# jgaeddert/liquid-usrp

Hardware: AMD Instinct MI355X
Metric: complex Msamples/s through multichannelrx (higher is better)
Workload: dtype f32

## Files before the change

### liquid-usrp_amd/csrc/lean_prims.hpp

```cpp
#pragma once
namespace lean {

typedef float v2f __attribute__((ext_vector_type(2)));
__device__ __forceinline__ v2f cmul_pk(v2f a, v2f tw)
{
    v2f t, r;
    asm("v_pk_mul_f32 %0, %1, %2 op_sel_hi:[1,0]" : "=v"(t) : "v"(a), "v"(tw));
    asm("v_pk_fma_f32 %0, %1, %2, %3 op_sel:[1,1,0] op_sel_hi:[0,1,1] neg_lo:[1,0,0]" : "=v"(r) : "v"(a), "v"(tw), "v"(t));
    return r;
}
__device__ __forceinline__ v2f cmulc_pk(v2f a, v2f tw)
{
    v2f t, r;
    asm("v_pk_mul_f32 %0, %1, %2 op_sel_hi:[1,0]" : "=v"(t) : "v"(a), "v"(tw));
    asm("v_pk_fma_f32 %0, %1, %2, %3 op_sel:[1,1,0] op_sel_hi:[0,1,1] neg_hi:[1,0,0]" : "=v"(r) : "v"(a), "v"(tw), "v"(t));
    return r;
}
__device__ __forceinline__ v2f rot_down_pk(v2f a, float rev)
{
    v2f cs; cs.x = __builtin_amdgcn_cosf(rev); cs.y = __builtin_amdgcn_sinf(rev);
    return cmulc_pk(a, cs);
}
template <int HI>
__device__ __forceinline__ v2f bfly_pk(v2f x, v2f sgp, v2f p)
{
    v2f r;
    if constexpr (HI == 0) asm("v_pk_fma_f32 %0, %1, %2, %3 op_sel_hi:[1,0,1]" : "=v"(r) : "v"(x), "v"(sgp), "v"(p));
    else                   asm("v_pk_fma_f32 %0, %1, %2, %3 op_sel:[0,1,0] op_sel_hi:[1,1,1]" : "=v"(r) : "v"(x), "v"(sgp), "v"(p));
    return r;
}

template <int H>
__device__ __forceinline__ float xch(float v, int bp32)
{
    if constexpr (H == 32) return __builtin_bit_cast(float, __builtin_amdgcn_ds_bpermute(bp32, __builtin_bit_cast(int, v)));
    else return __builtin_bit_cast(float, __builtin_amdgcn_ds_swizzle(__builtin_bit_cast(int, v), (H << 10) | 0x1F));
}
template <int H, int XB, int HI>
__device__ __forceinline__ v2f stage(v2f x, v2f sgp, v2f tw, int bp32)
{
    v2f u;
    if constexpr ((XB & H) != 0) { v2f p; p.x = xch<H>(x.x, bp32); p.y = xch<H>(x.y, bp32); u = bfly_pk<HI>(x, sgp, p); }
    else { const float sg = HI ? sgp.y : sgp.x; u.x = bfly_leg<H>(x.x, sg); u.y = bfly_leg<H>(x.y, sg); }
    if constexpr (H == 1) return u;
    else return cmul_pk(u, tw);
}


template <int MM> __device__ __forceinline__ int lane_k(int l)
{
    if constexpr (MM == 64) return (int)(__brev((unsigned)l) >> 26);
    else return l < 48 ? (l >> 4) + 3 * (int)(__brev((unsigned)(l & 15)) >> 28) : -1;
}
template <int MM> __device__ __forceinline__ int k_lane(int k)
{
    if constexpr (MM == 64) return (int)(__brev((unsigned)k) >> 26);
    else return 16 * (k % 3) + (int)(__brev((unsigned)(k / 3)) >> 28);
}
struct Radix3 { v2f w1, w2, t; int a0, a1, a2; };
__device__ __forceinline__ Radix3 radix3_consts(int l)
{
    Radix3 r;
    const int a = l >> 4, b = l & 15;
    const float r1 = (float)(a % 3) * (1.0f / 3.0f), r2 = (float)((2 * a) % 3) * (1.0f / 3.0f), rt = (float)(b * (a % 3)) * (1.0f / 48.0f);
    r.w1.x = __builtin_amdgcn_cosf(r1); r.w1.y = -__builtin_amdgcn_sinf(r1);
    r.w2.x = __builtin_amdgcn_cosf(r2); r.w2.y = -__builtin_amdgcn_sinf(r2);
    r.t.x = __builtin_amdgcn_cosf(rt);  r.t.y = -__builtin_amdgcn_sinf(rt);
    r.a0 = b << 2; r.a1 = (16 + b) << 2; r.a2 = (32 + b) << 2;
    return r;
}
template <int XB>
__device__ __forceinline__ v2f fft48(v2f x, const v2f (&tw)[6], const v2f (&sgp)[3], const Radix3 &r3, int bp32, int l)
{
    const float xr = x.x, xi = x.y;
    v2f x0, x1, x2;
    x0.x = __builtin_bit_cast(float, __builtin_amdgcn_ds_bpermute(r3.a0, __builtin_bit_cast(int, xr)));
    x0.y = __builtin_bit_cast(float, __builtin_amdgcn_ds_bpermute(r3.a0, __builtin_bit_cast(int, xi)));
    x1.x = __builtin_bit_cast(float, __builtin_amdgcn_ds_bpermute(r3.a1, __builtin_bit_cast(int, xr)));
    x1.y = __builtin_bit_cast(float, __builtin_amdgcn_ds_bpermute(r3.a1, __builtin_bit_cast(int, xi)));
    x2.x = __builtin_bit_cast(float, __builtin_amdgcn_ds_bpermute(r3.a2, __builtin_bit_cast(int, xr)));
    x2.y = __builtin_bit_cast(float, __builtin_amdgcn_ds_bpermute(r3.a2, __builtin_bit_cast(int, xi)));
    const v2f p1 = cmul_pk(x1, r3.w1), p2 = cmul_pk(x2, r3.w2);
    v2f y; y.x = (x0.x + p1.x) + p2.x; y.y = (x0.y + p1.y) + p2.y;
    y = cmul_pk(y, r3.t);
    if (l >= 48) { y.x = 0.f; y.y = 0.f; }
    y = stage<8, XB, 0>(y, sgp[1], tw[2], bp32);
    y = stage<4, XB, 1>(y, sgp[1], tw[3], bp32);
    y = stage<2, XB, 0>(y, sgp[2], tw[4], bp32);
    y = stage<1, XB, 1>(y, sgp[2], tw[5], bp32);
    return y;
}
template <int XB>
__device__ __forceinline__ v2f fft64(v2f x, const v2f (&tw)[6], const v2f (&sgp)[3], int bp32)
{
    x = stage<32, XB, 0>(x, sgp[0], tw[0], bp32);
    x = stage<16, XB, 1>(x, sgp[0], tw[1], bp32);
    x = stage<8, XB, 0>(x, sgp[1], tw[2], bp32);
    x = stage<4, XB, 1>(x, sgp[1], tw[3], bp32);
    x = stage<2, XB, 0>(x, sgp[2], tw[4], bp32);
    x = stage<1, XB, 1>(x, sgp[2], tw[5], bp32);
    return x;
}

}
```

### liquid-usrp_amd/csrc/payload_lean.hpp

```cpp

#ifndef PL_NT_STORE
#define PL_NT_STORE 0
#endif
#include "lean_prims.hpp"
#include "demod_pk.hpp"
namespace lean {

template <int MOD, int XB, int MM = 64>
__device__ __forceinline__ uint32_t symbols(const SyncArgs &a, const PayloadJob *job, const uint32_t ch, const uint32_t j,
                                            const uint32_t *qsg, const uint32_t *qnb, const int *qsrc)
{
    constexpr unsigned bps = bits_per_symbol<MOD>::v;
    const SyncConsts &c = a.c;
    const int l = lane_id();
    const int bp32 = (l ^ 32) << 2;
    const int kq = lane_k<MM>(l);
    const bool lane_on = kq >= 0;
    const int kk = lane_on ? kq : 0;
    const int dr = lane_on ? c.data_rank[kk] : -1;
    const bool isdata = dr >= 0;
    Radix3 r3; if constexpr (MM == 48) r3 = radix3_consts(l);
    const float fxr = ((kk > c.M2) ? (float)kk - (float)c.M : (float)kk) * 0.15915494309189535f;
    v2f R = {0.f, 0.f};
    if (lane_on && c.sctype[kk]) { const float2 g = (a.jR + (size_t)j * c.M)[kk]; R.x = g.x; R.y = g.y; }
    v2f tw[6], sgp[3];
#pragma unroll
    for (int st = 0; st < 6; st++) {
        const int h = 32 >> st;
        const bool up = (l & h) != 0;
        const float rev = (float)(l & (h - 1)) * (0.5f / (float)h);
        tw[st].x = up ? __builtin_amdgcn_cosf(rev) : 1.f; tw[st].y = up ? -__builtin_amdgcn_sinf(rev) : 0.f;
        if (st & 1) sgp[st >> 1].y = up ? -1.f : 1.f; else sgp[st >> 1].x = up ? -1.f : 1.f;
    }
    const int Mp = c.M_pilot;
    const bool p8 = Mp <= 8;
    const float pf0 = (l < Mp) ? c.Pfit[l] : 0.f, pf1 = (l < Mp) ? c.Pfit[Mp + l] : 0.f;
    const float pfc = p8 ? ((l < 8) ? pf0 : ((l < 16 && l - 8 < Mp) ? c.Pfit[Mp + l - 8] : 0.f)) : pf0;
    const int psrc = qsrc[l < Mp ? l : 0] << 2;
    const uint32_t so_sym = (uint32_t)(isdata ? dr : 0) * 8u, so_soft = (uint32_t)(isdata ? dr : 0) * bps;

    const int L = c.L, cb = c.cp - c.backoff, Md = c.M_data;
    const uint32_t mod_len = rfl(job->s.mod_len), nbits = rfl(8u * job->s.enc_len);
    const uint32_t nsym = (mod_len + (uint32_t)Md - 1u) / (uint32_t)Md;
    const int64_t t_ev0 = job->s.cur + (int64_t)job->s.timer - 1;
    const int64_t ws0 = t_ev0 - L + 1 + cb;
    uint32_t dth = rfl(job->s.nco_dtheta);
    uint32_t th_ws = rfl(job->s.nco_theta_ref + (uint32_t)(ws0 - job->s.nco_t_ref) * job->s.nco_dtheta);
    uint32_t pc4 = rfl(job->s.pilot_count) * 4u;
    float phi_prime = job->s.phi_prime, p1_prime = job->s.p1_prime;
    int32_t r_ws = (int32_t)rfl((uint32_t)(ws0 - a.buf_first));
    const float2 *chb = a.chan + ((size_t)a.chan_off + ch) * MCRX_TILE_S;
    const uint32_t tstride = a.chan_stride * (uint32_t)MCRX_TILE_S;
    const int32_t r_max = (int32_t)(a.end - a.buf_first) - 1;
    const bool soft_mode = c.payload_soft != 0;
    const bool keep_syms = a.no_syms == 0;
    uint8_t *soft = a.jsoft + (size_t)j * 8 * c.max_enc_len;
    const uint64_t syms_off = job->syms_off;
    uint8_t *syms = a.sarena + (((uint64_t)rfl((uint32_t)(syms_off >> 32)) << 32) | rfl((uint32_t)syms_off));
    const uint32_t l4 = (uint32_t)l * 4u;

    int q0 = -1, q1 = -1; uint32_t offl = 0, offl1 = 0;
    auto load_win = [&](int32_t rw) -> v2f {
        if (rw >= 0 && rw + (WV - 1) <= r_max) {
            const int ph = rw & (MCRX_TILE_S - 1);
            if (ph != q0) {
                const int tq = q0; const uint32_t to = offl; q0 = q1; offl = offl1; q1 = tq; offl1 = to;
                if (ph != q0) { q0 = ph; const uint32_t q = (uint32_t)ph + (uint32_t)l; offl = ((q >> MCRX_TILE_SH) * tstride + (q & (uint32_t)(MCRX_TILE_S - 1))) * 8u; }
            }
            const char *base = reinterpret_cast<const char *>(chb + (size_t)(uint32_t)(rw >> MCRX_TILE_SH) * tstride);
            v2f v = *reinterpret_cast<const v2f *>(base + offl);
            if constexpr (MM < WV) { if (l >= MM) { v.x = 0.f; v.y = 0.f; } }
            return v;
        }
        int32_t r = rw + l;
        r = r < 0 ? 0 : (r > r_max ? r_max : r);
        v2f v = *reinterpret_cast<const v2f *>(chb + ((size_t)(r >> MCRX_TILE_SH) * tstride + (size_t)(r & (MCRX_TILE_S - 1))));
        if constexpr (MM < WV) { if (l >= MM) { v.x = 0.f; v.y = 0.f; } }
        return v;
    };

    auto store_symbol = [&](uint32_t ps, v2f Z, uint64_t sw, bool inner) {
        uint8_t *ssym = syms + (size_t)ps * 8, *ssoft = soft + (size_t)ps * bps;
        if (inner || (ps + (uint32_t)Md <= mod_len && (ps + (uint32_t)Md) * bps <= nbits)) {
            if (isdata) {
#if PL_NT_STORE
                if (keep_syms) __builtin_nontemporal_store(Z, reinterpret_cast<v2f *>(ssym + so_sym));
#else
                if (keep_syms) *reinterpret_cast<v2f *>(ssym + so_sym) = Z;
#endif
                uint8_t *dst = ssoft + so_soft;
                if constexpr (bps == 1) dst[0] = (uint8_t)sw;
                else if constexpr (bps == 2) *reinterpret_cast<uint16_t *>(dst) = (uint16_t)sw;
                else {
                    *reinterpret_cast<uint16_t *>(dst) = (uint16_t)sw;
                    *reinterpret_cast<uint16_t *>(dst + 2) = (uint16_t)(sw >> 16);
                    if constexpr (bps == 6) *reinterpret_cast<uint16_t *>(dst + 4) = (uint16_t)(sw >> 32);
                }
            }
        } else if (isdata && ps + (uint32_t)dr < mod_len) {
            if (keep_syms) *reinterpret_cast<v2f *>(ssym + so_sym) = Z;
            const uint32_t b0 = (ps + (uint32_t)dr) * bps;
#pragma unroll
            for (unsigned kb = 0; kb < bps; kb++) if (b0 + kb < nbits) ssoft[so_soft + kb] = (uint8_t)(sw >> (8 * kb));
        }
    };
    v2f cur = load_win(r_ws);
    v2f Zp = {0.f, 0.f}; uint64_t swp = 0;
    uint32_t psi = 0;
    for (uint32_t n = 0; n < nsym; n++) {
        const uint32_t sgn = *reinterpret_cast<const uint32_t *>(reinterpret_cast<const char *>(qsg) + (pc4 + (l < 16 ? l4 : 0u)));
        v2f x = rot_down_pk(cur, u32rev(th_ws + (uint32_t)l * dth));
        if (n + 1 < nsym) cur = load_win(r_ws + L);
        if (n > 0) store_symbol(psi - (uint32_t)Md, Zp, swp, true);
        if constexpr (MM == 64) x = fft64<XB>(x, tw, sgp, bp32);
        else x = fft48<XB>(x, tw, sgp, r3, bp32, l);
        x = cmul_pk(x, R);
        const float xr = x.x, xi = x.y;
        float2 P;
        P.x = __builtin_bit_cast(float, __builtin_amdgcn_ds_bpermute(psrc, __builtin_bit_cast(int, xr)) ^ (int)sgn);
        P.y = __builtin_bit_cast(float, __builtin_amdgcn_ds_bpermute(psrc, __builtin_bit_cast(int, xi)) ^ (int)sgn);
        const float v = atan2_fast(P.y, P.x);
        const float prev = dpp_mov<0x111, false>(v, v);
        const float turns = rintf((v - prev) * 0.15915494309189535f);
        float p0, p1;
        if (p8) {
            float t = turns;
            t += dpp_mov<0x111>(t); t += dpp_mov<0x112>(t); t += dpp_mov<0x114>(t);
            const float y = fmaf(-TWO_PI_F, t, v);
            const int yi = __builtin_bit_cast(int, y);
            float z = pfc * __builtin_bit_cast(float, __builtin_amdgcn_update_dpp(yi, yi, 0x118, 0xf, 0xc, false));
            z += dpp_mov<0x111>(z); z += dpp_mov<0x112>(z); z += dpp_mov<0x114>(z);
            p0 = __builtin_bit_cast(float, __builtin_amdgcn_readlane(__builtin_bit_cast(int, z), 7));
            p1 = __builtin_bit_cast(float, __builtin_amdgcn_readlane(__builtin_bit_cast(int, z), 15));
        } else {
            const float y = fmaf(-TWO_PI_F, row_scan_fast(turns), v);
            p0 = row_total_dpp(pf0 * y);
            p1 = row_total_dpp(pf1 * y);
        }
        pc4 += (uint32_t)Mp * 4u; pc4 = pc4 >= 255u * 4u ? pc4 - 255u * 4u : pc4;
        p1 = 0.3f * p1 + (1.0f - 0.3f) * p1_prime;
        p1_prime = p1;
        Zp = rot_down_pk(x, fmaf(p1, fxr, p0 * 0.15915494309189535f));
        swp = demod_pk<MOD>(reinterpret_cast<const uint8_t *>(qnb), Zp, soft_mode);
        psi += (uint32_t)Md;
        float dphi = p0 - phi_prime;
        dphi -= TWO_PI_F * rintf(dphi * 0.15915494309189535f);
        phi_prime = p0;
        const uint32_t dnew = dth + rfl((uint32_t)__float2int_rn(dphi * (1e-3f * 683565275.5764316f)));
        th_ws += (uint32_t)(L - cb) * dth + (uint32_t)cb * dnew;
        dth = dnew;
        r_ws += L;
    }
    if (nsym > 0) store_symbol(psi - (uint32_t)Md, Zp, swp, false);
    return dth;
}

}

template <int XB, int CLS, bool REST = false, int MM = 64>
__device__ __forceinline__ void payload_lean_body(SyncArgs &a)
{
    launder(a);
    __shared__ uint32_t qsg[256 + 16];
    __shared__ uint32_t qnb[64];
    __shared__ int qsrc[16];
    const SyncConsts &c = a.c;
    const int l = lane_id();
    const uint32_t nj = a.max_jobs;
    uint32_t nlist = (CLS == 1 && a.qam_list) ? a.qam_list[0] : a.live[0];
    if (nlist > nj) nlist = nj;
    const uint32_t kfirst = REST ? a.live_off + blockIdx.x : blockIdx.x;
    if (kfirst >= nlist) return;
    for (int k = l; k < 256 + 16; k += WV) qsg[k] = c.pilot_seq[k >= 255 ? k - 255 : k] == 0 ? 0x80000000u : 0u;
    if (l < 16) qsrc[l] = 0;
    wave_sync_lds();
    { const int kq = lean::lane_k<MM>(l); const int pr = kq >= 0 ? c.pilot_rank[kq] : -1; if (pr >= 0 && pr < 16) qsrc[pr] = l; }
    wave_sync_lds();
    for (uint32_t k = kfirst; k < nlist; k += gridDim.x) {
        const uint32_t j = (CLS == 1 && a.qam_list) ? rfl(a.qam_list[1 + k]) : rfl(a.live[1 + k]);
        if (j >= nj) continue;
        const PayloadJob *job = a.jobs + j;
        const uint32_t ch = rfl(job->ch);
        if (ch >= a.nch || job->arena_off == ~0ull) continue;
        const uint32_t mod = rfl(job->s.mod_scheme);
        if (((mod == 39 || mod == 40) ? 0 : 1) != CLS) continue;
        uint32_t dth;
        if constexpr (CLS == 0) {
            if (mod == 39) dth = lean::symbols<39, XB, MM>(a, job, ch, j, qsg, qnb, qsrc);
            else           dth = lean::symbols<40, XB, MM>(a, job, ch, j, qsg, qnb, qsrc);
        } else {
            wave_sync_lds();
            if (mod == 27) { if (l < 16) qnb[l] = reinterpret_cast<const uint32_t *>(c.cod.qam16_nb)[l]; }
            else qnb[l] = reinterpret_cast<const uint32_t *>(c.cod.qam64_nb)[l];
            wave_sync_lds();
            if (mod == 27) dth = lean::symbols<27, XB, MM>(a, job, ch, j, qsg, qnb, qsrc);
            else           dth = lean::symbols<29, XB, MM>(a, job, ch, j, qsg, qnb, qsrc);
        }
        if (l == 0) a.jobs[j].s.nco_dtheta = dth;
        if (CLS == 0 && !REST) break;
    }
}
template <int XB, int MM = 64> __global__ __launch_bounds__(WV) __attribute__((amdgpu_num_sgpr(72))) void payload_lean_kernel(SyncArgs a) { payload_lean_body<XB, 0, false, MM>(a); }
template <int XB, int MM = 64> __global__ __launch_bounds__(WV) void payload_lean_rest_kernel(SyncArgs a) { payload_lean_body<XB, 0, true, MM>(a); payload_lean_body<XB, 1, false, MM>(a); }
```

### liquid-usrp_amd/csrc/payload_wide.hpp

```cpp
#include "lean_prims.hpp"
#include "demod_pk.hpp"
namespace lean {

template <int MOD, int XB, int E>
__device__ __forceinline__ uint32_t symbols_wide(const SyncArgs &a, const PayloadJob *job, const uint32_t ch, const uint32_t j,
                                                 const uint32_t *qsg, const uint32_t *qnb, const int *qsrc)
{
    constexpr unsigned bps = MOD == 39 ? 1u : MOD == 40 ? 2u : MOD == 27 ? 4u : 6u;
    constexpr int LOG2E = E == 2 ? 1 : (E == 4 ? 2 : 3);
    static_assert(E == 2 || E == 4 || E == 8, "symbol widths 128, 256, 512");
    const SyncConsts &c = a.c;
    const int l = lane_id();
    const int bp32 = (l ^ 32) << 2;
    int dr[E]; float fxr[E]; v2f R[E]; uint32_t so_sym[E], so_soft[E];
#pragma unroll
    for (int e = 0; e < E; e++) {
        const int kk = (int)(__brev((unsigned)(l + WV * e)) >> (32 - 6 - LOG2E));
        dr[e] = c.data_rank[kk];
        fxr[e] = ((kk > c.M2) ? (float)kk - (float)c.M : (float)kk) * 0.15915494309189535f;
        R[e].x = 0.f; R[e].y = 0.f;
        if (c.sctype[kk]) { const float2 g = (a.jR + (size_t)j * c.M)[kk]; R[e].x = g.x; R[e].y = g.y; }
        so_sym[e] = (uint32_t)(dr[e] >= 0 ? dr[e] : 0) * 8u; so_soft[e] = (uint32_t)(dr[e] >= 0 ? dr[e] : 0) * bps;
    }
    v2f tw[6], sgp[3];
#pragma unroll
    for (int st = 0; st < 6; st++) {
        const int h = 32 >> st;
        const bool up = (l & h) != 0;
        const float rev = (float)(l & (h - 1)) * (0.5f / (float)h);
        tw[st].x = up ? __builtin_amdgcn_cosf(rev) : 1.f; tw[st].y = up ? -__builtin_amdgcn_sinf(rev) : 0.f;
        if (st & 1) sgp[st >> 1].y = up ? -1.f : 1.f; else sgp[st >> 1].x = up ? -1.f : 1.f;
    }
    v2f itw[E - 1];
#pragma unroll
    for (int J = E / 2; J >= 1; J >>= 1)
#pragma unroll
        for (int r = 0; r < J; r++) {
            const float rev = (float)(l + WV * r) * (0.5f / (float)(WV * J));
            itw[J - 1 + r].x = __builtin_amdgcn_cosf(rev); itw[J - 1 + r].y = __builtin_amdgcn_sinf(rev);
        }
    const int Mp = c.M_pilot;
    const float pf0 = (l < Mp) ? c.Pfit[l] : 0.f, pf1 = (l < Mp) ? c.Pfit[Mp + l] : 0.f;
    const int psrc = qsrc[l < Mp ? l : 0];
    const int paddr = (psrc & 63) << 2, pel = psrc >> 8;

    const int L = c.L, cb = c.cp - c.backoff, Md = c.M_data;
    const uint32_t mod_len = rfl(job->s.mod_len), nbits = rfl(8u * job->s.enc_len);
    const uint32_t nsym = (mod_len + (uint32_t)Md - 1u) / (uint32_t)Md;
    const int64_t t_ev0 = job->s.cur + (int64_t)job->s.timer - 1;
    const int64_t ws0 = t_ev0 - L + 1 + cb;
    uint32_t dth = rfl(job->s.nco_dtheta);
    uint32_t th_ws = rfl(job->s.nco_theta_ref + (uint32_t)(ws0 - job->s.nco_t_ref) * job->s.nco_dtheta);
    uint32_t pc4 = rfl(job->s.pilot_count) * 4u;
    float phi_prime = job->s.phi_prime, p1_prime = job->s.p1_prime;
    int32_t r_ws = (int32_t)rfl((uint32_t)(ws0 - a.buf_first));
    const float2 *chb = a.chan + ((size_t)a.chan_off + ch) * MCRX_TILE_S;
    const uint32_t tstride = a.chan_stride * (uint32_t)MCRX_TILE_S;
    const int32_t r_max = (int32_t)(a.end - a.buf_first) - 1;
    const bool soft_mode = c.payload_soft != 0;
    const bool keep_syms = a.no_syms == 0;
    uint8_t *soft = a.jsoft + (size_t)j * 8 * c.max_enc_len;
    const uint64_t syms_off = job->syms_off;
    uint8_t *syms = a.sarena + (((uint64_t)rfl((uint32_t)(syms_off >> 32)) << 32) | rfl((uint32_t)syms_off));
    const uint32_t l4 = (uint32_t)l * 4u;

    int q0 = -1; uint32_t offl = 0;
    const uint32_t estep = (uint32_t)(WV >> MCRX_TILE_SH) * tstride * 8u;
    auto load_win = [&](int32_t rw, v2f (&w)[E]) {
        if (rw >= 0 && rw + (WV * E - 1) <= r_max) {
            const int ph = rw & (MCRX_TILE_S - 1);
            if (ph != q0) { q0 = ph; const uint32_t q = (uint32_t)ph + (uint32_t)l; offl = ((q >> MCRX_TILE_SH) * tstride + (q & (uint32_t)(MCRX_TILE_S - 1))) * 8u; }
            const char *base = reinterpret_cast<const char *>(chb + (size_t)(uint32_t)(rw >> MCRX_TILE_SH) * tstride) + offl;
#pragma unroll
            for (int e = 0; e < E; e++) w[e] = *reinterpret_cast<const v2f *>(base + (size_t)e * estep);
            return;
        }
#pragma unroll
        for (int e = 0; e < E; e++) {
            int32_t r = rw + l + WV * e;
            r = r < 0 ? 0 : (r > r_max ? r_max : r);
            w[e] = *reinterpret_cast<const v2f *>(chb + ((size_t)(r >> MCRX_TILE_SH) * tstride + (size_t)(r & (MCRX_TILE_S - 1))));
        }
    };
    auto store_symbol = [&](uint32_t ps, const v2f (&Z)[E], const uint64_t (&sw)[E], bool inner) {
        uint8_t *ssym = syms + (size_t)ps * 8, *ssoft = soft + (size_t)ps * bps;
        const bool whole = inner || (ps + (uint32_t)Md <= mod_len && (ps + (uint32_t)Md) * bps <= nbits);
#pragma unroll
        for (int e = 0; e < E; e++) {
            if (dr[e] < 0) continue;
            if (whole) {
                if (keep_syms) *reinterpret_cast<v2f *>(ssym + so_sym[e]) = Z[e];
                uint8_t *dst = ssoft + so_soft[e];
                if constexpr (bps == 1) dst[0] = (uint8_t)sw[e];
                else if constexpr (bps == 2) *reinterpret_cast<uint16_t *>(dst) = (uint16_t)sw[e];
                else if constexpr (bps == 4) *reinterpret_cast<uint32_t *>(dst) = (uint32_t)sw[e];
                else {
                    *reinterpret_cast<uint16_t *>(dst) = (uint16_t)sw[e];
                    *reinterpret_cast<uint16_t *>(dst + 2) = (uint16_t)(sw[e] >> 16);
                    *reinterpret_cast<uint16_t *>(dst + 4) = (uint16_t)(sw[e] >> 32);
                }
            } else if (ps + (uint32_t)dr[e] < mod_len) {
                if (keep_syms) *reinterpret_cast<v2f *>(ssym + so_sym[e]) = Z[e];
                const uint32_t b0 = (ps + (uint32_t)dr[e]) * bps;
#pragma unroll
                for (unsigned kb = 0; kb < bps; kb++) if (b0 + kb < nbits) ssoft[so_soft[e] + kb] = (uint8_t)(sw[e] >> (8 * kb));
            }
        }
    };
    v2f cur[E];
    load_win(r_ws, cur);
    v2f Zp[E]; uint64_t swp[E];
#pragma unroll
    for (int e = 0; e < E; e++) { Zp[e].x = 0.f; Zp[e].y = 0.f; swp[e] = 0; }
    uint32_t psi = 0;
    for (uint32_t n = 0; n < nsym; n++) {
        const uint32_t sgn = *reinterpret_cast<const uint32_t *>(reinterpret_cast<const char *>(qsg) + (pc4 + (l < Mp ? l4 : 0u)));
        v2f x[E];
#pragma unroll
        for (int e = 0; e < E; e++) x[e] = rot_down_pk(cur[e], u32rev(th_ws + (uint32_t)(l + WV * e) * dth));
        if (n + 1 < nsym) load_win(r_ws + L, cur);
        if (n > 0) store_symbol(psi - (uint32_t)Md, Zp, swp, true);
#pragma unroll
        for (int J = E / 2; J >= 1; J >>= 1)
#pragma unroll
            for (int e = 0; e < E; e++)
                if ((e & J) == 0) {
                    const v2f u = x[e], v = x[e + J];
                    x[e] = u + v;
                    x[e + J] = cmulc_pk(u - v, itw[J - 1 + (e & (J - 1))]);
                }
#pragma unroll
        for (int e = 0; e < E; e++) { x[e] = fft64<XB>(x[e], tw, sgp, bp32); x[e] = cmul_pk(x[e], R[e]); }
        float px = 0.f, py = 0.f;
#pragma unroll
        for (int e = 0; e < E; e++) {
            const float xr = x[e].x, xi = x[e].y;
            const int gx = __builtin_amdgcn_ds_bpermute(paddr, __builtin_bit_cast(int, xr)), gy = __builtin_amdgcn_ds_bpermute(paddr, __builtin_bit_cast(int, xi));
            if (pel == e) { px = __builtin_bit_cast(float, gx ^ (int)sgn); py = __builtin_bit_cast(float, gy ^ (int)sgn); }
        }
        const float v = atan2_fast(py, px);
        float p0, p1;
        if (Mp <= 16) {
            const float prev = dpp_mov<0x111, false>(v, v);
            const float turns = rintf((v - prev) * 0.15915494309189535f);
            const float y = fmaf(-TWO_PI_F, row_scan_fast(turns), v);
            p0 = row_total_dpp(pf0 * y);
            p1 = row_total_dpp(pf1 * y);
        } else {
            const float prev = dpp_mov<0x138, false>(v, v);
            const float turns = rintf((v - prev) * 0.15915494309189535f);
            const float y = fmaf(-TWO_PI_F, wave_scan_fast(turns), v);
            p0 = wave_total_dpp(pf0 * y);
            p1 = wave_total_dpp(pf1 * y);
        }
        pc4 += (uint32_t)Mp * 4u; pc4 = pc4 >= 255u * 4u ? pc4 - 255u * 4u : pc4;
        p1 = 0.3f * p1 + (1.0f - 0.3f) * p1_prime;
        p1_prime = p1;
        const float p0r = p0 * 0.15915494309189535f;
#pragma unroll
        for (int e = 0; e < E; e++) {
            Zp[e] = rot_down_pk(x[e], fmaf(p1, fxr[e], p0r));
            swp[e] = demod_pk<MOD>(reinterpret_cast<const uint8_t *>(qnb), Zp[e], soft_mode);
        }
        psi += (uint32_t)Md;
        float dphi = p0 - phi_prime;
        dphi -= TWO_PI_F * rintf(dphi * 0.15915494309189535f);
        phi_prime = p0;
        const uint32_t dnew = dth + rfl((uint32_t)__float2int_rn(dphi * (1e-3f * 683565275.5764316f)));
        th_ws += (uint32_t)(L - cb) * dth + (uint32_t)cb * dnew;
        dth = dnew;
        r_ws += L;
    }
    if (nsym > 0) store_symbol(psi - (uint32_t)Md, Zp, swp, false);
    return dth;
}

}

template <int XB, int E>
__global__ __launch_bounds__(WV, (E >= 4 ? 2 : 4)) void payload_wide_kernel(SyncArgs a)
{
    launder(a);
    __shared__ uint32_t qsg[256 + 64];
    __shared__ uint32_t qnb[64];
    __shared__ int qsrc[64];
    const SyncConsts &c = a.c;
    const int l = lane_id();
    const uint32_t nj = a.max_jobs;
    uint32_t nlist = a.live[0];
    if (nlist > nj) nlist = nj;
    if (blockIdx.x >= nlist) return;
    for (int k = l; k < 256 + 64; k += WV) qsg[k] = c.pilot_seq[k >= 255 ? k - 255 : k] == 0 ? 0x80000000u : 0u;
    qsrc[l] = 0;
    wave_sync_lds();
    constexpr int LOG2E = E == 2 ? 1 : (E == 4 ? 2 : 3);
#pragma unroll
    for (int e = 0; e < E; e++) {
        const int kk = (int)(__brev((unsigned)(l + WV * e)) >> (32 - 6 - LOG2E));
        const int pr = c.pilot_rank[kk];
        if (pr >= 0 && pr < 64) qsrc[pr] = (e << 8) | l;
    }
    wave_sync_lds();
    uint32_t mod_in_lds = 0;
    for (uint32_t k = blockIdx.x; k < nlist; k += gridDim.x) {
        const uint32_t j = rfl(a.live[1 + k]);
        if (j >= nj) continue;
        const PayloadJob *job = a.jobs + j;
        const uint32_t ch = rfl(job->ch);
        if (ch >= a.nch || job->arena_off == ~0ull) continue;
        const uint32_t mod = rfl(job->s.mod_scheme);
        if ((mod == 27 || mod == 29) && mod != mod_in_lds) {
            wave_sync_lds();
            if (mod == 27) { if (l < 16) qnb[l] = reinterpret_cast<const uint32_t *>(c.cod.qam16_nb)[l]; }
            else qnb[l] = reinterpret_cast<const uint32_t *>(c.cod.qam64_nb)[l];
            wave_sync_lds();
            mod_in_lds = mod;
        }
        uint32_t dth;
        if (mod == 39)      dth = lean::symbols_wide<39, XB, E>(a, job, ch, j, qsg, qnb, qsrc);
        else if (mod == 40) dth = lean::symbols_wide<40, XB, E>(a, job, ch, j, qsg, qnb, qsrc);
        else if (mod == 27) dth = lean::symbols_wide<27, XB, E>(a, job, ch, j, qsg, qnb, qsrc);
        else                dth = lean::symbols_wide<29, XB, E>(a, job, ch, j, qsg, qnb, qsrc);
        if (l == 0) a.jobs[j].s.nco_dtheta = dth;
    }
}
```

Measured before the change: 189,200.

## Add specialized two-symbol payload loop with incremental per-lane NCO phase

Adds a FIX-specialized path of the payload symbol loop for frames fully inside the buffer with soft mode on and at most eight pilots. It uses SGPR-based addressing for loads and stores, precomputed even/odd lane offsets, unchecked whole stores, and a loop unrolled over two symbols. Across both the lean and wide kernels, the NCO phase is now tracked incrementally per lane with a mad_i24 step and a scalar readfirstlane delta. The tile-offset multiply becomes a shift-add sum, and an s_nop barrier plus fp contract(off) pin instruction ordering and numerics. The goal is to cut per-symbol scalar, vector and branch overhead in the latency-bound loop. The cost is extra code size, more template instantiations, and the assumption that delta fits in 24-bit signed arithmetic.

```diff
diff --git a/liquid-usrp_amd/csrc/lean_prims.hpp b/liquid-usrp_amd/csrc/lean_prims.hpp
--- a/liquid-usrp_amd/csrc/lean_prims.hpp
+++ b/liquid-usrp_amd/csrc/lean_prims.hpp
@@ -19,6 +19,7 @@
 __device__ __forceinline__ v2f rot_down_pk(v2f a, float rev)
 {
     v2f cs; cs.x = __builtin_amdgcn_cosf(rev); cs.y = __builtin_amdgcn_sinf(rev);
+    asm("s_nop 0" : "+v"(cs));
     return cmulc_pk(a, cs);
 }
 template <int HI>
@@ -28,6 +29,39 @@
     if constexpr (HI == 0) asm("v_pk_fma_f32 %0, %1, %2, %3 op_sel_hi:[1,0,1]" : "=v"(r) : "v"(x), "v"(sgp), "v"(p));
     else                   asm("v_pk_fma_f32 %0, %1, %2, %3 op_sel:[0,1,0] op_sel_hi:[1,1,1]" : "=v"(r) : "v"(x), "v"(sgp), "v"(p));
     return r;
+}
+
+__device__ __forceinline__ uint32_t phase_step(uint32_t ph, uint32_t step, int k, int32_t delta)
+{
+    const uint32_t b = ph + step;
+    uint32_t r;
+    asm("v_mad_i32_i24 %0, %1, %2, %3" : "=v"(r) : "v"(k), "s"(delta), "v"(b));
+    return r;
+}
+__device__ __forceinline__ int32_t trim_sgpr(float dphi)
+{
+    int d = __float2int_rn(dphi * (1e-3f * 683565275.5764316f));
+    asm("" : "+v"(d));
+    return __builtin_amdgcn_readfirstlane(d);
+}
+
+__device__ __forceinline__ uint32_t small_times(uint32_t t, uint32_t m)
+{
+    return ((t & 1u) ? m : 0u) + ((t & 2u) ? 2u * m : 0u) + ((t & 4u) ? 4u * m : 0u);
+}
+template <typename T>
+__device__ __forceinline__ T gload_s(const void *base, uint32_t off)
+{
+    uint64_t v = reinterpret_cast<uint64_t>(base);
+    asm("" : "+s"(v), "+v"(off));
+    return *(const __attribute__((address_space(1))) T *)(v + off);
+}
+template <typename T>
+__device__ __forceinline__ void gstore_s(void *base, uint32_t off, T val)
+{
+    uint64_t v = reinterpret_cast<uint64_t>(base);
+    asm("" : "+s"(v), "+v"(off));
+    *(__attribute__((address_space(1))) T *)(v + off) = val;
 }
 
 template <int H>
diff --git a/liquid-usrp_amd/csrc/payload_lean.hpp b/liquid-usrp_amd/csrc/payload_lean.hpp
--- a/liquid-usrp_amd/csrc/payload_lean.hpp
+++ b/liquid-usrp_amd/csrc/payload_lean.hpp
@@ -6,7 +6,19 @@
 #include "demod_pk.hpp"
 namespace lean {
 
-template <int MOD, int XB, int MM = 64>
+__device__ __forceinline__ bool frame_inside(const SyncArgs &a, const PayloadJob *job)
+{
+    const SyncConsts &c = a.c;
+    const int L = c.L, cb = c.cp - c.backoff, Md = c.M_data;
+    const uint32_t mod_len = rfl(job->s.mod_len);
+    const uint32_t nsym = (mod_len + (uint32_t)Md - 1u) / (uint32_t)Md;
+    const int64_t ws0 = job->s.cur + (int64_t)job->s.timer - 1 - L + 1 + cb;
+    const int32_t r_ws = (int32_t)rfl((uint32_t)(ws0 - a.buf_first));
+    const int32_t r_max = (int32_t)(a.end - a.buf_first) - 1;
+    return ((2 * L) & (MCRX_TILE_S - 1)) == 0 && nsym > 0 && r_ws >= 0 && (int64_t)r_ws + (int64_t)nsym * L + (WV - 1) <= (int64_t)r_max;
+}
+
+template <int MOD, int XB, int MM = 64, bool FIX = false>
 __device__ __forceinline__ uint32_t symbols(const SyncArgs &a, const PayloadJob *job, const uint32_t ch, const uint32_t j,
                                             const uint32_t *qsg, const uint32_t *qnb, const int *qsrc)
 {
@@ -33,7 +45,7 @@
         if (st & 1) sgp[st >> 1].y = up ? -1.f : 1.f; else sgp[st >> 1].x = up ? -1.f : 1.f;
     }
     const int Mp = c.M_pilot;
-    const bool p8 = Mp <= 8;
+    const bool p8 = FIX ? true : Mp <= 8;
     const float pf0 = (l < Mp) ? c.Pfit[l] : 0.f, pf1 = (l < Mp) ? c.Pfit[Mp + l] : 0.f;
     const float pfc = p8 ? ((l < 8) ? pf0 : ((l < 16 && l - 8 < Mp) ? c.Pfit[Mp + l - 8] : 0.f)) : pf0;
     const int psrc = qsrc[l < Mp ? l : 0] << 2;
@@ -45,30 +57,38 @@
     const int64_t t_ev0 = job->s.cur + (int64_t)job->s.timer - 1;
     const int64_t ws0 = t_ev0 - L + 1 + cb;
     uint32_t dth = rfl(job->s.nco_dtheta);
-    uint32_t th_ws = rfl(job->s.nco_theta_ref + (uint32_t)(ws0 - job->s.nco_t_ref) * job->s.nco_dtheta);
+    const uint32_t th_ws0 = rfl(job->s.nco_theta_ref + (uint32_t)(ws0 - job->s.nco_t_ref) * job->s.nco_dtheta);
+    uint32_t ph_l = th_ws0 + (uint32_t)l * dth;
     uint32_t pc4 = rfl(job->s.pilot_count) * 4u;
     float phi_prime = job->s.phi_prime, p1_prime = job->s.p1_prime;
     int32_t r_ws = (int32_t)rfl((uint32_t)(ws0 - a.buf_first));
     const float2 *chb = a.chan + ((size_t)a.chan_off + ch) * MCRX_TILE_S;
     const uint32_t tstride = a.chan_stride * (uint32_t)MCRX_TILE_S;
     const int32_t r_max = (int32_t)(a.end - a.buf_first) - 1;
-    const bool soft_mode = c.payload_soft != 0;
-    const bool keep_syms = a.no_syms == 0;
+    const bool soft_mode = FIX ? true : c.payload_soft != 0;
+    const bool keep_syms = FIX ? true : a.no_syms == 0;
     uint8_t *soft = a.jsoft + (size_t)j * 8 * c.max_enc_len;
     const uint64_t syms_off = job->syms_off;
     uint8_t *syms = a.sarena + (((uint64_t)rfl((uint32_t)(syms_off >> 32)) << 32) | rfl((uint32_t)syms_off));
     const uint32_t l4 = (uint32_t)l * 4u;
 
+    const uint32_t lt_off = (uint32_t)(l >> MCRX_TILE_SH) * tstride;
+    auto lane_off = [&](int ph) -> uint32_t {
+        const uint32_t q = (uint32_t)ph + (uint32_t)(l & (MCRX_TILE_S - 1));
+        return (lt_off + ((q >> MCRX_TILE_SH) ? tstride : 0u) + (q & (uint32_t)(MCRX_TILE_S - 1))) * 8u;
+    };
+    auto win_base = [&](int32_t rw) -> const char * {
+        return reinterpret_cast<const char *>(chb + (size_t)(uint32_t)(rw >> MCRX_TILE_SH) * tstride);
+    };
     int q0 = -1, q1 = -1; uint32_t offl = 0, offl1 = 0;
     auto load_win = [&](int32_t rw) -> v2f {
         if (rw >= 0 && rw + (WV - 1) <= r_max) {
             const int ph = rw & (MCRX_TILE_S - 1);
             if (ph != q0) {
                 const int tq = q0; const uint32_t to = offl; q0 = q1; offl = offl1; q1 = tq; offl1 = to;
-                if (ph != q0) { q0 = ph; const uint32_t q = (uint32_t)ph + (uint32_t)l; offl = ((q >> MCRX_TILE_SH) * tstride + (q & (uint32_t)(MCRX_TILE_S - 1))) * 8u; }
-            }
-            const char *base = reinterpret_cast<const char *>(chb + (size_t)(uint32_t)(rw >> MCRX_TILE_SH) * tstride);
-            v2f v = *reinterpret_cast<const v2f *>(base + offl);
+                if (ph != q0) { q0 = ph; offl = lane_off(ph); }
+            }
+            v2f v = *reinterpret_cast<const v2f *>(win_base(rw) + offl);
             if constexpr (MM < WV) { if (l >= MM) { v.x = 0.f; v.y = 0.f; } }
             return v;
         }
@@ -79,39 +99,36 @@
         return v;
     };
 
+    auto store_whole = [&](uint8_t *ssym, uint8_t *ssoft, v2f Z, uint64_t sw) {
+        if (isdata) {
+#if PL_NT_STORE
+            if (keep_syms) __builtin_nontemporal_store(Z, reinterpret_cast<v2f *>(ssym + so_sym));
+#else
+            if (keep_syms) *reinterpret_cast<v2f *>(ssym + so_sym) = Z;
+#endif
+            uint8_t *dst = ssoft + so_soft;
+            if constexpr (bps == 1) dst[0] = (uint8_t)sw;
+            else if constexpr (bps == 2) *reinterpret_cast<uint16_t *>(dst) = (uint16_t)sw;
+            else {
+                *reinterpret_cast<uint16_t *>(dst) = (uint16_t)sw;
+                *reinterpret_cast<uint16_t *>(dst + 2) = (uint16_t)(sw >> 16);
+                if constexpr (bps == 6) *reinterpret_cast<uint16_t *>(dst + 4) = (uint16_t)(sw >> 32);
+            }
+        }
+    };
     auto store_symbol = [&](uint32_t ps, v2f Z, uint64_t sw, bool inner) {
         uint8_t *ssym = syms + (size_t)ps * 8, *ssoft = soft + (size_t)ps * bps;
-        if (inner || (ps + (uint32_t)Md <= mod_len && (ps + (uint32_t)Md) * bps <= nbits)) {
-            if (isdata) {
-#if PL_NT_STORE
-                if (keep_syms) __builtin_nontemporal_store(Z, reinterpret_cast<v2f *>(ssym + so_sym));
-#else
-                if (keep_syms) *reinterpret_cast<v2f *>(ssym + so_sym) = Z;
-#endif
-                uint8_t *dst = ssoft + so_soft;
-                if constexpr (bps == 1) dst[0] = (uint8_t)sw;
-                else if constexpr (bps == 2) *reinterpret_cast<uint16_t *>(dst) = (uint16_t)sw;
-                else {
-                    *reinterpret_cast<uint16_t *>(dst) = (uint16_t)sw;
-                    *reinterpret_cast<uint16_t *>(dst + 2) = (uint16_t)(sw >> 16);
-                    if constexpr (bps == 6) *reinterpret_cast<uint16_t *>(dst + 4) = (uint16_t)(sw >> 32);
-                }
-            }
-        } else if (isdata && ps + (uint32_t)dr < mod_len) {
+        if (inner || (ps + (uint32_t)Md <= mod_len && (ps + (uint32_t)Md) * bps <= nbits)) store_whole(ssym, ssoft, Z, sw);
+        else if (isdata && ps + (uint32_t)dr < mod_len) {
             if (keep_syms) *reinterpret_cast<v2f *>(ssym + so_sym) = Z;
             const uint32_t b0 = (ps + (uint32_t)dr) * bps;
 #pragma unroll
             for (unsigned kb = 0; kb < bps; kb++) if (b0 + kb < nbits) ssoft[so_soft + kb] = (uint8_t)(sw >> (8 * kb));
         }
     };
-    v2f cur = load_win(r_ws);
     v2f Zp = {0.f, 0.f}; uint64_t swp = 0;
     uint32_t psi = 0;
-    for (uint32_t n = 0; n < nsym; n++) {
-        const uint32_t sgn = *reinterpret_cast<const uint32_t *>(reinterpret_cast<const char *>(qsg) + (pc4 + (l < 16 ? l4 : 0u)));
-        v2f x = rot_down_pk(cur, u32rev(th_ws + (uint32_t)l * dth));
-        if (n + 1 < nsym) cur = load_win(r_ws + L);
-        if (n > 0) store_symbol(psi - (uint32_t)Md, Zp, swp, true);
+    auto finish = [&](v2f x, uint32_t sgn) {
         if constexpr (MM == 64) x = fft64<XB>(x, tw, sgp, bp32);
         else x = fft48<XB>(x, tw, sgp, r3, bp32, l);
         x = cmul_pk(x, R);
@@ -138,7 +155,10 @@
             p1 = row_total_dpp(pf1 * y);
         }
         pc4 += (uint32_t)Mp * 4u; pc4 = pc4 >= 255u * 4u ? pc4 - 255u * 4u : pc4;
-        p1 = 0.3f * p1 + (1.0f - 0.3f) * p1_prime;
+        {
+#pragma clang fp contract(off)
+            p1 = 0.3f * p1 + (1.0f - 0.3f) * p1_prime;
+        }
         p1_prime = p1;
         Zp = rot_down_pk(x, fmaf(p1, fxr, p0 * 0.15915494309189535f));
         swp = demod_pk<MOD>(reinterpret_cast<const uint8_t *>(qnb), Zp, soft_mode);
@@ -146,13 +166,50 @@
         float dphi = p0 - phi_prime;
         dphi -= TWO_PI_F * rintf(dphi * 0.15915494309189535f);
         phi_prime = p0;
-        const uint32_t dnew = dth + rfl((uint32_t)__float2int_rn(dphi * (1e-3f * 683565275.5764316f)));
-        th_ws += (uint32_t)(L - cb) * dth + (uint32_t)cb * dnew;
+        const int32_t delta = trim_sgpr(dphi);
+        const uint32_t dnew = dth + (uint32_t)delta;
+        ph_l = phase_step(ph_l, (uint32_t)(L - cb) * dth + (uint32_t)cb * dnew, l, delta);
         dth = dnew;
         r_ws += L;
+    };
+
+    if constexpr (FIX) {
+        static_assert(MM == WV && bps <= 2, "the two-symbol loop: 64-sample windows, BPSK / QPSK");
+        v2f cur = gload_s<v2f>(win_base(r_ws), lane_off(r_ws & (MCRX_TILE_S - 1)));
+        const uint32_t off_even = lane_off(r_ws & (MCRX_TILE_S - 1)), off_odd = lane_off((r_ws + L) & (MCRX_TILE_S - 1));
+        uint8_t *ssym = syms, *ssoft = soft;
+        auto symbol = [&](auto has_prev, const uint32_t off_next) {
+            const uint32_t sgn = *reinterpret_cast<const uint32_t *>(reinterpret_cast<const char *>(qsg) + (pc4 + (l < 16 ? l4 : 0u)));
+            const v2f x = rot_down_pk(cur, u32rev(ph_l));
+            cur = gload_s<v2f>(win_base(r_ws + L), off_next);
+            if constexpr (decltype(has_prev)::value) {
+                if (isdata) {
+                    if (keep_syms) gstore_s<v2f>(ssym, so_sym, Zp);
+                    if constexpr (bps == 1) gstore_s<uint8_t>(ssoft, so_soft, (uint8_t)swp);
+                    else gstore_s<uint16_t>(ssoft, so_soft, (uint16_t)swp);
+                }
+                ssym += (size_t)Md * 8; ssoft += (size_t)Md * bps;
+            }
+            finish(x, sgn);
+        };
+        symbol(std::false_type{}, off_odd);
+        uint32_t n = 1;
+        for (; n + 2 <= nsym; n += 2) { symbol(std::true_type{}, off_even); symbol(std::true_type{}, off_odd); }
+        if (n < nsym) symbol(std::true_type{}, off_even);
+        store_symbol(psi - (uint32_t)Md, Zp, swp, false);
+        return dth;
+    } else {
+    v2f cur = load_win(r_ws);
+    for (uint32_t n = 0; n < nsym; n++) {
+        const uint32_t sgn = *reinterpret_cast<const uint32_t *>(reinterpret_cast<const char *>(qsg) + (pc4 + (l < 16 ? l4 : 0u)));
+        const v2f x = rot_down_pk(cur, u32rev(ph_l));
+        if (n + 1 < nsym) cur = load_win(r_ws + L);
+        if (n > 0) store_symbol(psi - (uint32_t)Md, Zp, swp, true);
+        finish(x, sgn);
     }
     if (nsym > 0) store_symbol(psi - (uint32_t)Md, Zp, swp, false);
     return dth;
+    }
 }
 
 }
@@ -184,10 +241,14 @@
         if (ch >= a.nch || job->arena_off == ~0ull) continue;
         const uint32_t mod = rfl(job->s.mod_scheme);
         if (((mod == 39 || mod == 40) ? 0 : 1) != CLS) continue;
-        uint32_t dth;
+        uint32_t dth = 0;
         if constexpr (CLS == 0) {
-            if (mod == 39) dth = lean::symbols<39, XB, MM>(a, job, ch, j, qsg, qnb, qsrc);
-            else           dth = lean::symbols<40, XB, MM>(a, job, ch, j, qsg, qnb, qsrc);
+            bool fix = false;
+            if constexpr (MM == 64) fix = c.M_pilot <= 8 && c.payload_soft != 0 && a.no_syms == 0 && lean::frame_inside(a, job);
+            if constexpr (MM == 64) {
+                if (fix) dth = mod == 39 ? lean::symbols<39, XB, MM, true>(a, job, ch, j, qsg, qnb, qsrc) : lean::symbols<40, XB, MM, true>(a, job, ch, j, qsg, qnb, qsrc);
+            }
+            if (!fix) dth = mod == 39 ? lean::symbols<39, XB, MM>(a, job, ch, j, qsg, qnb, qsrc) : lean::symbols<40, XB, MM>(a, job, ch, j, qsg, qnb, qsrc);
         } else {
             wave_sync_lds();
             if (mod == 27) { if (l < 16) qnb[l] = reinterpret_cast<const uint32_t *>(c.cod.qam16_nb)[l]; }
diff --git a/liquid-usrp_amd/csrc/payload_wide.hpp b/liquid-usrp_amd/csrc/payload_wide.hpp
--- a/liquid-usrp_amd/csrc/payload_wide.hpp
+++ b/liquid-usrp_amd/csrc/payload_wide.hpp
@@ -50,7 +50,8 @@
     const int64_t t_ev0 = job->s.cur + (int64_t)job->s.timer - 1;
     const int64_t ws0 = t_ev0 - L + 1 + cb;
     uint32_t dth = rfl(job->s.nco_dtheta);
-    uint32_t th_ws = rfl(job->s.nco_theta_ref + (uint32_t)(ws0 - job->s.nco_t_ref) * job->s.nco_dtheta);
+    const uint32_t th_ws0 = rfl(job->s.nco_theta_ref + (uint32_t)(ws0 - job->s.nco_t_ref) * job->s.nco_dtheta);
+    uint32_t ph_l = th_ws0 + (uint32_t)l * dth;
     uint32_t pc4 = rfl(job->s.pilot_count) * 4u;
     float phi_prime = job->s.phi_prime, p1_prime = job->s.p1_prime;
     int32_t r_ws = (int32_t)rfl((uint32_t)(ws0 - a.buf_first));
@@ -69,7 +70,7 @@
     auto load_win = [&](int32_t rw, v2f (&w)[E]) {
         if (rw >= 0 && rw + (WV * E - 1) <= r_max) {
             const int ph = rw & (MCRX_TILE_S - 1);
-            if (ph != q0) { q0 = ph; const uint32_t q = (uint32_t)ph + (uint32_t)l; offl = ((q >> MCRX_TILE_SH) * tstride + (q & (uint32_t)(MCRX_TILE_S - 1))) * 8u; }
+            if (ph != q0) { q0 = ph; const uint32_t q = (uint32_t)ph + (uint32_t)l; offl = (small_times(q >> MCRX_TILE_SH, tstride) + (q & (uint32_t)(MCRX_TILE_S - 1))) * 8u; }
             const char *base = reinterpret_cast<const char *>(chb + (size_t)(uint32_t)(rw >> MCRX_TILE_SH) * tstride) + offl;
 #pragma unroll
             for (int e = 0; e < E; e++) w[e] = *reinterpret_cast<const v2f *>(base + (size_t)e * estep);
@@ -117,7 +118,7 @@
         const uint32_t sgn = *reinterpret_cast<const uint32_t *>(reinterpret_cast<const char *>(qsg) + (pc4 + (l < Mp ? l4 : 0u)));
         v2f x[E];
 #pragma unroll
-        for (int e = 0; e < E; e++) x[e] = rot_down_pk(cur[e], u32rev(th_ws + (uint32_t)(l + WV * e) * dth));
+        for (int e = 0; e < E; e++) x[e] = rot_down_pk(cur[e], u32rev(ph_l + (uint32_t)(WV * e) * dth));
         if (n + 1 < nsym) load_win(r_ws + L, cur);
         if (n > 0) store_symbol(psi - (uint32_t)Md, Zp, swp, true);
 #pragma unroll
@@ -166,8 +167,9 @@
         float dphi = p0 - phi_prime;
         dphi -= TWO_PI_F * rintf(dphi * 0.15915494309189535f);
         phi_prime = p0;
-        const uint32_t dnew = dth + rfl((uint32_t)__float2int_rn(dphi * (1e-3f * 683565275.5764316f)));
-        th_ws += (uint32_t)(L - cb) * dth + (uint32_t)cb * dnew;
+        const int32_t delta = trim_sgpr(dphi);
+        const uint32_t dnew = dth + (uint32_t)delta;
+        ph_l = phase_step(ph_l, (uint32_t)(L - cb) * dth + (uint32_t)cb * dnew, l, delta);
         dth = dnew;
         r_ws += L;
     }
```

After: 192,600, median of 6. 1.02x the previous value.
